# jmduarte/gnn-fpga

Hardware: AMD Instinct MI355X
Metric: edges/sec (EdgeNet+NodeNet fwd) on 100k-edge TrackML graphs; % HBM roofline (higher is better)
Workload: dtype f32; 1 GPU; c3 synthetic TrackML ACTS graphs: 256 graphs/launch/GPU x (10k hits, 100k segments), F=3, D=8, 3 MP iterations + final edge pass, index form resident in HBM; graphs_per_gpu=256, hits_per_graph=10000, segments_per_graph=100000

## Files before the change

gnn-fpga_amd/csrc/sell_pipeline.hip:

```cpp
#include "common.h"

#include <cstdlib>
#include <type_traits>
#include <utility>

namespace {
using namespace gnn;

constexpr int SLICE = 16;
constexpr int DESC = 8;

template <int F, int D>
struct TL {
    static constexpr int d4 = D / 4, C = F + D;
    static constexpr int a4(int x) { return (x + 3) & ~3; }
    static constexpr int o_w2 = 0;
    static constexpr int o_in = a4(o_w2 + d4);
    static constexpr int in_sz = d4 + F * d4;
    static constexpr int o_4 = a4(o_in + in_sz);
    static constexpr int w4_sz = d4 + D * d4;
    static constexpr int o_m = a4(o_4 + w4_sz);
    static constexpr int m_sz = d4 + C * d4;
    static constexpr int m_st = a4(m_sz);
    static constexpr int o_b2 = o_m + 5 * m_st;
// ... 40 lines not shown
            const int k = (t - d4) / d4, i = (t - d4) % d4;
            v = p.W4[(q * d4 + i) * D + k];
        }
    } else if (pos >= L::o_m && pos < L::o_b2 && (pos - L::o_m) % L::m_st < L::m_sz) {
        const int t = pos - L::o_m, m = t / L::m_st, u = t % L::m_st;
        if (u < d4) {
            const int r = q * d4 + u;
            v = (m == 0) ? kTwoLog2e * p.b1[r] : (m == 4) ? p.b3[r] : 0.0f;
        } else {
            const int k = (u - d4) / d4, r = q * d4 + (u - d4) % d4;
            switch (m) {
            case 0: v = kTwoLog2e * p.W1[r * 2 * C + k]; break;
            case 1: v = p.W3[r * 3 * C + k]; break;
            case 2: v = kTwoLog2e * p.W1[r * 2 * C + C + k]; break;
            case 3: v = p.W3[r * 3 * C + C + k]; break;
            default: v = p.W3[r * 3 * C + 2 * C + k]; break;
            }
        }
    } else if (pos == L::o_b2) {
        float sw = p.b2[0];
        for (int k = 0; k < D; ++k) sw += p.W2[k];
        v = -kLog2e * sw;
    }
    return v;
}

template <int F, int D, bool XP>
__device__ __forceinline__ void write_null_rows(const gnn_params_t &p, float *PRa, float *PRb,
                                                float *QSa, float *QSb, float *U, float *Pc,
                                                float *Qc, int64_t n_hits)
{
    constexpr int d4 = D / 4;
    for (int t = threadIdx.x; t < 2 * D; t += 256) {
        const int q = t / (2 * d4), w = t % (2 * d4);
        float pv = (w < d4) ? kTwoLog2e * p.b1[q * d4 + w] : 0.0f;
        if (XP && w < d4) pv = __builtin_amdgcn_exp2f(pv);
        const float qv = (XP && w < d4) ? 1.0f : 0.0f;
        PRa[n_hits * 2 * D + t] = pv;
        PRb[n_hits * 2 * D + t] = pv;
        QSa[n_hits * 2 * D + t] = qv;
        QSb[n_hits * 2 * D + t] = qv;
    }
    for (int t = threadIdx.x; t < D; t += 256) {
        U[n_hits * D + t] = 0.0f;
        const float pb = kTwoLog2e * p.b1[t];
        Pc[n_hits * D + t] = XP ? __builtin_amdgcn_exp2f(pb) : pb;
        Qc[n_hits * D + t] = XP ? 1.0f : 0.0f;
    }
}

template <int F, int D, bool XP>
__global__ __launch_bounds__(256) void k_pack(gnn_params_t p, float *__restrict__ table,
                                              float *PRa, float *PRb, float *QSa, float *QSb,
                                              float *U, float *Pc, float *Qc, int64_t n_hits)
{
    using L = TL<F, D>;
    for (int idx = blockIdx.x * 256 + threadIdx.x; idx < L::total; idx += gridDim.x * 256)
        table[idx] = table_entry<F, D>(p, idx);
    if (blockIdx.x == 0) write_null_rows<F, D, XP>(p, PRa, PRb, QSa, QSb, U, Pc, Qc, n_hits);
}

template <int CTRL>
__device__ __forceinline__ float dpp(float v)
{
    return __builtin_bit_cast(
        float, __builtin_amdgcn_mov_dpp(__builtin_bit_cast(int, v), CTRL, 0xF, 0xF, true));
}

__device__ __forceinline__ float quad_sum(float v)
{
    v += dpp<0xB1>(v);
    v += dpp<0x4E>(v);
    return v;
}

template <int N>
__device__ __forceinline__ void quad_allgather(const float (&loc)[N], float *out)
{
#pragma unroll
    for (int i = 0; i < N; ++i) {
        out[0 * N + i] = dpp<0x00>(loc[i]);
        out[1 * N + i] = dpp<0x55>(loc[i]);
        out[2 * N + i] = dpp<0xAA>(loc[i]);
        out[3 * N + i] = dpp<0xFF>(loc[i]);
    }
}

template <int N>
__device__ __forceinline__ void load_vec(const float *__restrict__ src, float *dst)
{
    if constexpr (N == 1) {
        dst[0] = src[0];
    } else if constexpr (N == 2) {
        const float2 v = *reinterpret_cast<const float2 *>(src);
        dst[0] = v.x; dst[1] = v.y;
    } else {
        static_assert(N % 4 == 0, "vector length");
#pragma unroll
        for (int i = 0; i < N / 4; ++i) {
            const float4 v = reinterpret_cast<const float4 *>(src)[i];
            dst[4 * i] = v.x; dst[4 * i + 1] = v.y; dst[4 * i + 2] = v.z; dst[4 * i + 3] = v.w;
        }
    }
}

typedef float f2_t __attribute__((ext_vector_type(2)));
typedef float f3_t __attribute__((ext_vector_type(3)));
typedef float f4_t __attribute__((ext_vector_type(4)));

template <int N>
__device__ __forceinline__ void store_vec(float *__restrict__ dst, const float *src)
{
    if constexpr (N == 1) {
        dst[0] = src[0];
    } else if constexpr (N == 2) {
        *reinterpret_cast<float2 *>(dst) = make_float2(src[0], src[1]);
    } else {
        static_assert(N % 4 == 0, "vector length");
#pragma unroll
        for (int i = 0; i < N / 4; ++i)
            reinterpret_cast<float4 *>(dst)[i] =
                make_float4(src[4 * i], src[4 * i + 1], src[4 * i + 2], src[4 * i + 3]);
    }
}

template <int NT>
__device__ __forceinline__ void stage4(const float *__restrict__ g, float *lds, int n4)
{
    const float4 *__restrict__ g4 = reinterpret_cast<const float4 *>(g);
    float4 *l4 = reinterpret_cast<float4 *>(lds);
    int i = threadIdx.x;
    for (; i + 7 * NT < n4; i += 8 * NT) {
        float4 v[8];
#pragma unroll
        for (int j = 0; j < 8; ++j) v[j] = g4[i + j * NT];
#pragma unroll
        for (int j = 0; j < 8; ++j) l4[i + j * NT] = v[j];
    }
    for (; i < n4; i += NT) l4[i] = g4[i];
}

template <int F, int D>
struct Cfg {
    static constexpr int NT = (D <= 16) ? 1024 : 256;
    static constexpr int lds_bytes = 160 * 1024;
    static constexpr int table_bytes = TL<F, D>::total * 4;
    static constexpr bool wide16 = (D == 16 && F <= 4);
    static constexpr int it_rec = (D <= 16 && !wide16) ? (lds_bytes - table_bytes - 2048) / (8 * D) : 0;
    static constexpr int ed_rec = (D <= 16) ? (lds_bytes - 2048) / (4 * D) : 0;
    static constexpr int tile_hits = (D <= 16 && !wide16) ? 1280 : 256;
    static constexpr int chunk_segments = 16384;
    static constexpr bool pipelined = (D <= 8 && F <= 3) || (D == 4);
    static constexpr bool iter2 = (D <= 8);
    static constexpr bool pack_first = (TL<F, D>::total > 4096);
    static constexpr bool fuse_first = iter2 && F <= 3 && !(F == 2 && D == 8);
};

template <int D4, int KD, int KF, bool PK = true>
__device__ __forceinline__ void role_gemv(const float *w, const float *hn, const float *x,
                                          float *out)
{
    constexpr int NW = D4 + (KD + KF) * D4;
    constexpr int CH = 8;
#ifndef GNN_NO_GEMV_PK
    if constexpr (PK && D4 >= 8 && D4 % 4 == 0) {
        const f4_t *wv = reinterpret_cast<const f4_t *>(__builtin_assume_aligned(w, 16));
        asm volatile("" ::: "memory");
        f2_t o2[D4 / 2];
#pragma unroll
        for (int v = 0; v < D4 / 4; ++v) {
            const f4_t t = wv[v];
            o2[2 * v] = f2_t{t.x, t.y};
            o2[2 * v + 1] = f2_t{t.z, t.w};
        }
        f4_t cur[D4 / 4], nxt[D4 / 4];
#pragma unroll
        for (int v = 0; v < D4 / 4; ++v) cur[v] = wv[D4 / 4 + v];
#pragma unroll
        for (int k = 0; k < KD + KF; ++k) {
            if (k + 1 < KD + KF)
#pragma unroll
                for (int v = 0; v < D4 / 4; ++v) nxt[v] = wv[(D4 + (k + 1) * D4) / 4 + v];
            const float in = k < KD ? hn[k < KD ? k : 0] : x[k >= KD ? k - KD : 0];
            const f2_t in2 = {in, in};
#pragma unroll
            for (int v = 0; v < D4 / 4; ++v) {
                o2[2 * v] = f2_t{cur[v].x, cur[v].y} * in2 + o2[2 * v];
                o2[2 * v + 1] = f2_t{cur[v].z, cur[v].w} * in2 + o2[2 * v + 1];
            }
#pragma unroll
            for (int v = 0; v < D4 / 4; ++v) cur[v] = nxt[v];
        }
#pragma unroll
        for (int i = 0; i < D4 / 2; ++i) {
            out[2 * i] = o2[i].x;
            out[2 * i + 1] = o2[i].y;
        }
        return;
    }
#endif
    const float4 *w4 = reinterpret_cast<const float4 *>(__builtin_assume_aligned(w, 16));
#pragma unroll
    for (int c0 = 0; c0 < NW; c0 += CH) {
        constexpr int dummy = 0; (void)dummy;
        float wr[CH];
#pragma unroll
        for (int v = 0; v < CH / 4; ++v) {
            if (c0 + 4 * v < NW) {
                const float4 t = w4[c0 / 4 + v];
                wr[4 * v] = t.x; wr[4 * v + 1] = t.y; wr[4 * v + 2] = t.z; wr[4 * v + 3] = t.w;
            }
        }
#pragma unroll
        for (int j = 0; j < CH; ++j) {
            const int g = c0 + j;
            if (g < NW) {
                if (g < D4) {
                    out[g] = wr[j];
                } else {
                    const int k = (g - D4) / D4, i = (g - D4) % D4;
                    out[i] = fmaf(wr[j], k < KD ? hn[k < KD ? k : 0] : x[k >= KD ? k - KD : 0], out[i]);
                }
            }
        }
    }
}

template <int KD, int KF>
__device__ __forceinline__ void role_gemv_burst(const float *w, const float *hn, const float *x,
                                                float *out)
{
    constexpr int NW = 2 + (KD + KF) * 2, NV = (NW + 3) / 4;
    const f4_t *wv = reinterpret_cast<const f4_t *>(__builtin_assume_aligned(w, 16));
    f4_t t[NV];
#pragma unroll
    for (int v = 0; v < NV; ++v) t[v] = wv[v];
    f2_t acc = {t[0].x, t[0].y};
#pragma unroll
    for (int j = 1; j < NW / 2; ++j) {
        const int k = j - 1;
        const float in = k < KD ? hn[k < KD ? k : 0] : x[k >= KD ? k - KD : 0];
        const f2_t wk = (j & 1) ? f2_t{t[j / 2].z, t[j / 2].w} : f2_t{t[j / 2].x, t[j / 2].y};
        acc = wk * f2_t{in, in} + acc;
    }
    out[0] = acc.x;
    out[1] = acc.y;
}

template <int F, int D, bool LAST, bool XP>
struct Records {
    static constexpr int d4 = D / 4;
    float pr[LAST ? d4 : 2 * d4], qs[LAST ? d4 : 2 * d4], u[d4];

    __device__ __forceinline__ void compute(const float *wl, const float *hn, const float *x)
    {
        using L = TL<F, D>;
        if constexpr (LAST) {
            role_gemv<d4, D, F>(wl + L::o_m + 0 * L::m_st, hn, x, pr);
            role_gemv<d4, D, F>(wl + L::o_m + 2 * L::m_st, hn, x, qs);
        } else {
            role_gemv<d4, D, F>(wl + L::o_m + 0 * L::m_st, hn, x, pr);
            role_gemv<d4, D, F>(wl + L::o_m + 1 * L::m_st, hn, x, pr + d4);
            role_gemv<d4, D, F>(wl + L::o_m + 2 * L::m_st, hn, x, qs);
            role_gemv<d4, D, F>(wl + L::o_m + 3 * L::m_st, hn, x, qs + d4);
            role_gemv<d4, D, F>(wl + L::o_m + 4 * L::m_st, hn, x, u);
        }
        if constexpr (XP) {
#pragma unroll
            for (int i = 0; i < d4; ++i) {
                pr[i] = __builtin_amdgcn_exp2f(pr[i]);
                qs[i] = __builtin_amdgcn_exp2f(qs[i]);
            }
        }
    }
    __device__ __forceinline__ void store(int64_t n, int q, float *__restrict__ PRn,
                                          float *__restrict__ QSn, float *__restrict__ U,
                                          float *__restrict__ Pc, float *__restrict__ Qc) const
    {
        if constexpr (LAST) {
            store_vec<d4>(Pc + n * D + q * d4, pr);
            store_vec<d4>(Qc + n * D + q * d4, qs);
        } else {
            store_vec<2 * d4>(PRn + n * 2 * D + q * 2 * d4, pr);
            store_vec<2 * d4>(QSn + n * 2 * D + q * 2 * d4, qs);
            store_vec<d4>(U + n * D + q * d4, u);
        }
    }
};

template <int F, int D, bool LAST, bool XP, bool PK = true>
__device__ __forceinline__ void emit_to(const float *wl, const float *hn, const float *x,
                                        float *__restrict__ pr_dst, float *__restrict__ qs_dst,
                                        float *__restrict__ u_dst)
{
    using L = TL<F, D>;
    constexpr int d4 = D / 4;
    {
        float pr[LAST ? d4 : 2 * d4];
        role_gemv<d4, D, F, PK>(wl + L::o_m + 0 * L::m_st, hn, x, pr);
        if constexpr (XP)
#pragma unroll
            for (int i = 0; i < d4; ++i) pr[i] = __builtin_amdgcn_exp2f(pr[i]);
        if constexpr (!LAST) role_gemv<d4, D, F, PK>(wl + L::o_m + 1 * L::m_st, hn, x, pr + d4);
        store_vec<LAST ? d4 : 2 * d4>(pr_dst, pr);
    }
    {
// ... 694 lines not shown
}
template <int J>
__device__ __forceinline__ float quad_bcast_f(float v)
{
    return dpp<J * 0x55>(v);
}

constexpr int MAXC = 6;

template <int D>
struct Recs {
    float r[4][2 * (D / 4)];
    __device__ __forceinline__ void read(int cur, const float *REC, int q)
    {
        constexpr int d4 = D / 4;
        const int nb[4] = {quad_bcast_i<0>(cur), quad_bcast_i<1>(cur), quad_bcast_i<2>(cur),
                           quad_bcast_i<3>(cur)};
#ifdef GNN_ABLATE_LDS
#pragma unroll
        for (int j = 0; j < 4; ++j)
#pragma unroll
            for (int i = 0; i < 2 * d4; ++i) r[j][i] = __int_as_float(nb[j] + i);
        (void)REC;
#else
#pragma unroll
        for (int j = 0; j < 4; ++j) load_vec<2 * d4>(REC + (int64_t)nb[j] * 2 * D + q * 2 * d4, r[j]);
#endif
    }
};

__device__ __forceinline__ float bf_lo(unsigned w) { return __uint_as_float(w << 16); }
__device__ __forceinline__ float bf_hi(unsigned w) { return __uint_as_float(w & 0xFFFF0000u); }

template <int D4, bool XP, bool ES = false>
__device__ __forceinline__ void score4(const float (*rec)[2 * D4], const float *own,
                                       const float *w2, float b2, int q, float *acc, float *eo = nullptr,
                                       bool ok = false)
{
    float part[4];
#ifndef GNN_NO_PK
    constexpr bool use_pk = (D4 == 2), use_pk_wide = (D4 >= 8 && D4 % 2 == 0);
#else
    constexpr bool use_pk = false, use_pk_wide = false;
#endif
    if constexpr (use_pk) {
        const f2_t o2 = {own[0], own[1]}, one2 = {1.0f, 1.0f};
        float r[4][2];
#pragma unroll
        for (int j = 0; j < 4; ++j) {
            const f2_t pj = {rec[j][0], rec[j][1]};
            f2_t a;
            if constexpr (XP) {
                a = pj * o2 + one2;
            } else {
                const f2_t z = pj + o2;
                const f2_t ex = {__builtin_amdgcn_exp2f(z.x), __builtin_amdgcn_exp2f(z.y)};
                a = ex + one2;
            }
            r[j][0] = __builtin_amdgcn_rcpf(a.x);
            r[j][1] = __builtin_amdgcn_rcpf(a.y);
        }
        const f2_t wa = {w2[0], w2[0]}, wb = {w2[1], w2[1]};
        const f2_t p01 = wa * f2_t{r[0][0], r[1][0]} + wb * f2_t{r[0][1], r[1][1]};
        const f2_t p23 = wa * f2_t{r[2][0], r[3][0]} + wb * f2_t{r[2][1], r[3][1]};
        part[0] = p01.x; part[1] = p01.y; part[2] = p23.x; part[3] = p23.y;
    } else if constexpr (use_pk_wide) {
        const f2_t one2 = {1.0f, 1.0f};
#pragma unroll
        for (int j = 0; j < 4; ++j) {
            f2_t pj = {0.0f, 0.0f};
#pragma unroll
            for (int i = 0; i < D4; i += 2) {
                const f2_t rj = {rec[j][i], rec[j][i + 1]}, o2 = {own[i], own[i + 1]};
                f2_t a;
                if constexpr (XP) {
                    a = rj * o2 + one2;
                } else {
                    const f2_t z = rj + o2;
                    const f2_t ex = {__builtin_amdgcn_exp2f(z.x), __builtin_amdgcn_exp2f(z.y)};
                    a = ex + one2;
                }
                const f2_t r = {__builtin_amdgcn_rcpf(a.x), __builtin_amdgcn_rcpf(a.y)};
                pj = f2_t{w2[i], w2[i + 1]} * r + pj;
            }
            part[j] = pj.x + pj.y;
        }
    } else {
#pragma unroll
        for (int j = 0; j < 4; ++j) {
            part[j] = 0.0f;
#pragma unroll
            for (int i = 0; i < D4; ++i) {
                const float r = XP ? __builtin_amdgcn_rcpf(fmaf(rec[j][i], own[i], 1.0f))
                                   : r_f(rec[j][i] + own[i]);
                part[j] = fmaf(w2[i], r, part[j]);
            }
        }
    }
    const bool odd = q & 1, hi = q & 2;
    const float s0 = odd ? part[0] : part[1], s1 = odd ? part[2] : part[3];
    const float k0 = odd ? part[1] : part[0], k1 = odd ? part[3] : part[2];
    const float t0 = k0 + dpp<0xB1>(s0), t1 = k1 + dpp<0xB1>(s1);
    const float give = hi ? t0 : t1, keep = hi ? t1 : t0;
    const float mine = keep + dpp<0x4E>(give);
    const float e = r_f(mine + b2);
    if constexpr (ES)
        if (ok) *eo = e;
    const float e4[4] = {quad_bcast_f<0>(e), quad_bcast_f<1>(e), quad_bcast_f<2>(e),
                         quad_bcast_f<3>(e)};
    if constexpr (use_pk_wide) {
#pragma unroll
        for (int j = 0; j < 4; ++j) {
            const f2_t e2 = {e4[j], e4[j]};
#pragma unroll
            for (int i = 0; i < D4; i += 2) {
                const f2_t a2 = f2_t{rec[j][D4 + i], rec[j][D4 + i + 1]} * e2 + f2_t{acc[i], acc[i + 1]};
                acc[i] = a2.x;
                acc[i + 1] = a2.y;
            }
        }
    } else {
#pragma unroll
        for (int j = 0; j < 4; ++j)
#pragma unroll
            for (int i = 0; i < D4; ++i) acc[i] = fmaf(e4[j], rec[j][D4 + i], acc[i]);
    }
}

template <int D, bool XP, bool ES = false>
__device__ __forceinline__ void sweep(const int *pre, const int32_t *__restrict__ lst, int len,
                                      int null_idx, const float *REC, int q, const float *own,
                                      const float *w2, float b2, float *acc, float *ebase = nullptr, int elen = 0)
{
    constexpr int d4 = D / 4;
    if (len <= 0) return;
    auto fix = [&](int cur, int rem) {
        const int lim = rem < 4 ? rem : 4;
        return (q < lim) ? cur : null_idx;
    };
    Recs<D> a;
#pragma unroll
    for (int c = 0; c < MAXC; ++c) {
        if (4 * c < len) {
            a.read(fix(pre[c], len - 4 * c), REC, q);
            score4<d4, XP, ES>(a.r, own, w2, b2, q, acc, ebase + 4 * c + q, 4 * c + q < elen);
        }
    }
    for (int k = 4 * MAXC; k < len; k += 4) {
        a.read(fix(lst[k * SLICE], len - k), REC, q);
        score4<d4, XP, ES>(a.r, own, w2, b2, q, acc, ebase + k + q, k + q < elen);
    }
}

template <int D, int NC, bool XP, bool PIPE>
__device__ __forceinline__ void sweep16(int (&c)[NC], const int32_t *__restrict__ nbr16,
                                        const int32_t *__restrict__ off16, int slice, int i16,
                                        int len, const float *REC, int q, const float *own,
                                        const float *w2, float b2, float *acc)
{
    constexpr int d4 = D / 4;
    if (len <= 0) return;
    int taken = 0;
    auto take_word = [&]() {
        int w = c[0];
        if (taken >= NC) {
            a_load_i32_s<0>(w, nbr16 + __builtin_amdgcn_readfirstlane(off16[slice]) + taken * 4 * SLICE,
                            (unsigned)(q * SLICE + i16) * 4u);
            a_wait_all();
            asm volatile("" : "+v"(w));
        }
#pragma unroll
        for (int i = 0; i + 1 < NC; ++i) c[i] = c[i + 1];
        ++taken;
        return w;
    };
    typedef __attribute__((address_space(3))) const float lds_cf;
    const unsigned rec0 = (unsigned)(uintptr_t)(lds_cf *)(REC + q * 2 * d4);
    auto issue = [&](float (*r)[2 * d4], int w, bool hi) {
        const int wa = hi ? quad_bcast_i<2>(w) : quad_bcast_i<0>(w);
        const int wb = hi ? quad_bcast_i<3>(w) : quad_bcast_i<1>(w);
        unsigned ad[4];
        static_assert(8 * D <= 64, "record size must be an inline constant");
        asm("v_mad_u32_u16 %0, %1, %2, %3" : "=v"(ad[0]) : "v"(wa), "n"(8 * D), "v"(rec0));
        asm("v_mad_u32_u16 %0, %1, %2, %3 op_sel:[1,0,0,0]" : "=v"(ad[1]) : "v"(wa), "n"(8 * D), "v"(rec0));
        asm("v_mad_u32_u16 %0, %1, %2, %3" : "=v"(ad[2]) : "v"(wb), "n"(8 * D), "v"(rec0));
        asm("v_mad_u32_u16 %0, %1, %2, %3 op_sel:[1,0,0,0]" : "=v"(ad[3]) : "v"(wb), "n"(8 * D), "v"(rec0));
#pragma unroll
        for (int j = 0; j < 4; ++j) {
            if constexpr (d4 == 2) {
                const f4_t v = *(const __attribute__((address_space(3))) f4_t *)(uintptr_t)ad[j];
                r[j][0] = v.x; r[j][1] = v.y; r[j][2] = v.z; r[j][3] = v.w;
            } else {
                const f2_t v = *(const __attribute__((address_space(3))) f2_t *)(uintptr_t)ad[j];
                r[j][0] = v.x; r[j][1] = v.y;
            }
        }
    };
    static_assert(d4 == 1 || d4 == 2, "record piece is 8 or 16 bytes");
    if constexpr (!PIPE) {
        for (int k = 0; k < len; k += 8) {
            const int w = take_word();
            float r[4][2 * d4];
            issue(r, w, false);
            score4<d4, XP>(r, own, w2, b2, q, acc);
            if (k + 4 < len) {
                issue(r, w, true);
                score4<d4, XP>(r, own, w2, b2, q, acc);
            }
        }
        return;
    }
    float ra[4][2 * d4], rb[4][2 * d4];
    int w = take_word();
    issue(ra, w, false);
    for (int k = 0; k < len; k += 8) {
        const bool has_hi = k + 4 < len;
        if (has_hi) issue(rb, w, true);
        score4<d4, XP>(ra, own, w2, b2, q, acc);
        if (has_hi) {
            if (k + 8 < len) {
                w = take_word();
                issue(ra, w, false);
            }
            score4<d4, XP>(rb, own, w2, b2, q, acc);
        }
    }
}

struct TrainOut {
    const int32_t *seg_ptr;
    float *e_t, *Q_t, *H_next;
    int ldh;
};

template <int F, int D, bool LAST, bool XP, bool TR = false>
__global__ __launch_bounds__((Cfg<F, D>::NT)) void k_iter(
    const float *__restrict__ X, const float *__restrict__ table,
    const int32_t *__restrict__ tiles, const int32_t *__restrict__ in_off,
    const int32_t *__restrict__ in_nbr, const int32_t *__restrict__ out_off,
    const int32_t *__restrict__ out_nbr, const float *__restrict__ PR,
    const float *__restrict__ QS, float *__restrict__ U, float *__restrict__ PRn,
    float *__restrict__ QSn, float *__restrict__ Pc, float *__restrict__ Qc, int64_t n_pad,
    int tiles_per_xcd, int n_tiles, int ablate, TrainOut tro = TrainOut{})
{
    using L = TL<F, D>;
    using G = Cfg<F, D>;
    constexpr int d4 = L::d4, NT = G::NT;
    (void)tro;
    extern __shared__ __attribute__((aligned(16))) float smem[];
    float *lds = smem, *win = smem + L::total;
    stage4<NT>(table, lds, L::total / 4);

    const int tile = (blockIdx.x & 7) * tiles_per_xcd + (blockIdx.x >> 3);
    if (tile >= n_tiles) return;
    const int32_t *td = tiles + (int64_t)tile * DESC;
    const int s_begin = td[0], s_end = td[1], in_lo = td[2], in_cnt = td[3], out_lo = td[4],
              out_cnt = td[5], mode = td[6];
    const int lane = threadIdx.x & 63;
    const int q = lane & 3, i16 = lane >> 2;

    struct Pre {
        int il, ol, ib, ob;
        int cin[MAXC], cout[MAXC];
        AVec<d4> Pn, Qn;
        AVec<d4> acc;
        AVec<F> x;
    };
    auto prefetch = [&](Pre &p, int slice) {
        if (ablate & 8) { p.il = 12; p.ol = 12; p.ib = 0; p.ob = 0;
#pragma unroll
            for (int c = 0; c < MAXC; ++c) { p.cin[c] = 0; p.cout[c] = 0; }
            return; }
        p.ib = __builtin_amdgcn_readfirstlane(in_off[slice]);
        p.il = (__builtin_amdgcn_readfirstlane(in_off[slice + 1]) - p.ib) >> 4;
        p.ob = __builtin_amdgcn_readfirstlane(out_off[slice]);
        p.ol = (__builtin_amdgcn_readfirstlane(out_off[slice + 1]) - p.ob) >> 4;
        const int32_t *li = in_nbr + p.ib + q * SLICE + i16;
        const int32_t *lo = out_nbr + p.ob + q * SLICE + i16;
#define GNN_PF(C_)                                                              \
        if (4 * C_ < p.il) a_load_i32<C_ * 4 * SLICE * 4>(p.cin[C_], li);           \
        if (4 * C_ < p.ol) a_load_i32<C_ * 4 * SLICE * 4>(p.cout[C_], lo);
        GNN_PF(0) GNN_PF(1) GNN_PF(2) GNN_PF(3) GNN_PF(4) GNN_PF(5)
#undef GNN_PF
        static_assert(MAXC == 6, "prefetch is written out for 6 chunks");
        const int64_t n = (int64_t)slice * SLICE + i16;
        p.Pn.load(PR + n * 2 * D + q * 2 * d4);
        p.Qn.load(QS + n * 2 * D + q * 2 * d4);
        p.acc.load(U + n * D + q * d4);
        p.x.load(X + n * F);
    };
    auto arrive = [&](Pre &p) {
        a_wait_all();
        a_fence(p.cin); a_fence(p.cout);
        p.Pn.fence(); p.Qn.fence(); p.acc.fence(); p.x.fence();
    };
    constexpr int NWV = NT / 64;
    const int wv = threadIdx.x >> 6;
    const int rounds = (s_end - s_begin + NWV - 1) / NWV;
    auto slice_of = [&](int r) {
        const int sl = s_begin + r * NWV + ((r & 1) ? NWV - 1 - wv : wv);
        return (r < rounds && sl < s_end) ? sl : -1;
    };
    Pre cur, nxt;
    int slice = slice_of(0);
    if (slice >= 0) prefetch(cur, slice);
    float *winA = win, *winB = win + (in_cnt + 1) * 2 * D;
    if (G::it_rec > 0 && mode && !(ablate & 1)) {
        stage4<NT>(PR + (int64_t)in_lo * 2 * D, winA, in_cnt * 2 * D / 4);
        stage4<NT>(PR + n_pad * 2 * D, winA + in_cnt * 2 * D, 2 * D / 4);
        stage4<NT>(QS + (int64_t)out_lo * 2 * D, winB, out_cnt * 2 * D / 4);
        stage4<NT>(QS + n_pad * 2 * D, winB + out_cnt * 2 * D, 2 * D / 4);
    }
    __syncthreads();
    if (slice >= 0) arrive(cur);
    float w2[d4];
#pragma unroll
    for (int i = 0; i < d4; ++i) w2[i] = lds[q * L::stride + L::o_w2 + i];
    const float b2 = lds[L::o_b2];

    for (int r = 0; r < rounds; ++r) {
        const int next = slice_of(r + 1);
        if (next >= 0) {
            prefetch(nxt, next);
            if constexpr (!G::pipelined || TR) arrive(nxt);
        }
        Records<F, D, LAST, XP> rec;
        const int64_t n = (int64_t)slice * SLICE + i16;
        if (slice >= 0) {
            int woff = q * L::stride;
            asm volatile("" : "+v"(woff));
            const float *wl = lds + woff;
            float acc[d4], Pn[d4], Qn[d4], xv[F];
            cur.acc.get(acc); cur.x.get(xv);
            cur.Pn.get(Pn); cur.Qn.get(Qn);
            float *eb = nullptr;
            int en = 0;
            if constexpr (TR) {
                const int s0 = tro.seg_ptr[n];
                en = tro.seg_ptr[n + 1] - s0;
                eb = tro.e_t + s0;
            }
            if (ablate & 2) {
            } else if (G::it_rec > 0 && mode) {
                sweep<D, XP, TR>(cur.cin, in_nbr + cur.ib + q * SLICE + i16, cur.il, in_cnt, winA, q, Qn, w2, b2, acc, eb, en);
                sweep<D, XP>(cur.cout, out_nbr + cur.ob + q * SLICE + i16, cur.ol, out_cnt, winB, q, Pn, w2, b2, acc);
            } else {
                sweep<D, XP, TR>(cur.cin, in_nbr + cur.ib + q * SLICE + i16, cur.il, (int)n_pad, PR, q, Qn, w2, b2, acc, eb, en);
                sweep<D, XP>(cur.cout, out_nbr + cur.ob + q * SLICE + i16, cur.ol, (int)n_pad, QS, q, Pn, w2, b2, acc);
            }
            float ql[d4], qa[D];
#pragma unroll
            for (int i = 0; i < d4; ++i) ql[i] = tanh_f(acc[i]);
            if constexpr (TR) store_vec<d4>(tro.Q_t + n * D + q * d4, ql);
            quad_allgather<d4>(ql, qa);
            float hl[d4];
            role_gemv<d4, D, 0>(wl + L::o_4, qa, qa, hl);
#pragma unroll
            for (int i = 0; i < d4; ++i) hl[i] = tanh_f(hl[i]);
            if constexpr (TR) {
                float *hr = tro.H_next + n * tro.ldh;
                store_vec<d4>(hr + q * d4, hl);
                if (q == 0) {
#pragma unroll
                    for (int k = 0; k < F; ++k) hr[D + k] = xv[k];
                    for (int k = D + F; k < tro.ldh; ++k) hr[k] = 0.0f;
                }
            }
            float hn[D];
            quad_allgather<d4>(hl, hn);
            if (!(ablate & 4)) rec.compute(wl, hn, xv);
        }
        if constexpr (G::pipelined)
            if (next >= 0) arrive(nxt);
        cur = nxt;
        if (slice >= 0 && !(ablate & 16)) rec.store(n, q, PRn, QSn, U, Pc, Qc);
        slice = next;
    }
}

// ... 767 lines not shown
#pragma unroll
            for (int k = 0; k < F; ++k) x[k] = live ? xb[h * F + k] : 0.0f;
            round_fence(r);
            if (!live) continue;
            h0_of(wl, x, hn);
            if constexpr (d4 == 2) {
                role_gemv_burst<D, F>(wl + L::o_m + (2 * M) * L::m_st, hn, x, rec);
                role_gemv_burst<D, F>(wl + L::o_m + (2 * M + 1) * L::m_st, hn, x, rec + d4);
            } else {
                role_gemv<d4, D, F>(wl + L::o_m + (2 * M) * L::m_st, hn, x, rec);
                role_gemv<d4, D, F>(wl + L::o_m + (2 * M + 1) * L::m_st, hn, x, rec + d4);
            }
            if constexpr (XP)
#pragma unroll
                for (int i = 0; i < d4; ++i) rec[i] = __builtin_amdgcn_exp2f(rec[i]);
            store_vec<2 * d4>(buf + h * 2 * D + q * 2 * d4, rec);
        }
        null_fence();
        put_null(buf, cnt, which);
    };

    struct PreA0 { int len; int c[NC]; AVec<d4> Q, U; };
    constexpr bool XPRE = F <= 4;
    struct PreB0 { int len; int c[NC]; AVec<d4> P; AVec<XPRE ? F : 0> x; };
    struct PreX { int len; int c[NC]; AVec<F> x; };
    using PreA = std::conditional_t<FIRST, PreX, PreA0>;
    using PreB = std::conditional_t<FIRST, PreX, PreB0>;
    const unsigned lo_list = (unsigned)(q * SLICE + i16) * 4u;
    const unsigned lo_rec = (unsigned)(i16 * 2 * D + q * 2 * d4) * 4u;
    const unsigned lo_vec = (unsigned)(i16 * D + q * d4) * 4u;
    const unsigned lo_x = (unsigned)(i16 * F) * 4u;
    auto prefetchA = [&](PreA &p, int slice_) {
        const int slice = __builtin_amdgcn_readfirstlane(slice_);
        p.len = (__builtin_amdgcn_readfirstlane(in_off[slice + 1]) -
                 __builtin_amdgcn_readfirstlane(in_off[slice])) >> 4;
        const int32_t *li = in_nbr16 + __builtin_amdgcn_readfirstlane(in_off16[slice]);
#define GNN_PF(C_) if (8 * C_ < p.len) a_load_i32_s<C_ * 4 * SLICE * 4>(p.c[C_], li, lo_list);
        GNN_PF(0) GNN_PF(1) GNN_PF(2)
#undef GNN_PF
        const int64_t n0 = (int64_t)slice * SLICE;
        if constexpr (FIRST) {
            p.x.load_s(X + n0 * F, lo_x);
        } else {
            p.Q.load_s(QS + n0 * 2 * D, lo_rec);
            p.U.load_s(U + n0 * D, lo_vec);
        }
    };
    auto prefetchB = [&](PreB &p, int slice_) {
        const int slice = __builtin_amdgcn_readfirstlane(slice_);
        p.len = (__builtin_amdgcn_readfirstlane(out_off[slice + 1]) -
                 __builtin_amdgcn_readfirstlane(out_off[slice])) >> 4;
        const int32_t *lo = out_nbr16 + __builtin_amdgcn_readfirstlane(out_off16[slice]);
#define GNN_PF(C_) if (8 * C_ < p.len) a_load_i32_s<C_ * 4 * SLICE * 4>(p.c[C_], lo, lo_list);
        GNN_PF(0) GNN_PF(1) GNN_PF(2)
#undef GNN_PF
        static_assert(NC == 3, "prefetch is written out for 3 words (24 steps)");
        const int64_t n0 = (int64_t)slice * SLICE;
        if constexpr (!FIRST) p.P.load_s(PR + n0 * 2 * D, lo_rec);
        if constexpr (XPRE || FIRST) p.x.load_s(X + n0 * F, lo_x);
    };
    auto arriveA = [&](PreA &p) {
        a_wait_all();
        a_fence(p.c);
        if constexpr (FIRST) {
            p.x.fence();
        } else {
            p.Q.fence();
            p.U.fence();
        }
    };
    auto arriveB = [&](PreB &p) {
        a_wait_all();
        a_fence(p.c);
        if constexpr (!FIRST) p.P.fence();
        if constexpr (XPRE || FIRST) p.x.fence();
    };

    constexpr int MAXR = 5;
    float ac0[d4], ac1[d4], ac2[d4], ac3[d4], ac4[d4];
    auto acc_put = [&](int r, const float *a) {
#pragma unroll
        for (int i = 0; i < d4; ++i) {
            ac0[i] = (r == 0) ? a[i] : ac0[i];
            ac1[i] = (r == 1) ? a[i] : ac1[i];
            ac2[i] = (r == 2) ? a[i] : ac2[i];
            ac3[i] = (r == 3) ? a[i] : ac3[i];
            ac4[i] = (r >= 4) ? a[i] : ac4[i];
        }
    };
    auto acc_get = [&](int r, float *a) {
#pragma unroll
        for (int i = 0; i < d4; ++i)
            a[i] = (r == 0) ? ac0[i] : (r == 1) ? ac1[i] : (r == 2) ? ac2[i] : (r == 3) ? ac3[i] : ac4[i];
    };
    static_assert(MAXR == 5, "accumulator slots are written out for 5 rounds");
#pragma unroll
    for (int i = 0; i < d4; ++i) ac0[i] = ac1[i] = ac2[i] = ac3[i] = ac4[i] = 0.0f;

    Desc d = load_desc(tile);
    PreA a_cur, a_nxt;
    PreB b_cur, b_nxt;
    if constexpr (FIRST) {
        xstage_issue(d.in_lo, d.in_cnt, bufA, capA);
        if (slice_a(d, 0) >= 0) prefetchA(a_cur, slice_a(d, 0));
        compute_window(bufA, d.in_cnt, capA, WinA{});
    } else {
        stage_issue(PR + (int64_t)d.in_lo * 2 * D, bufA, d.in_cnt);
        if (slice_a(d, 0) >= 0) prefetchA(a_cur, slice_a(d, 0));
        __syncthreads();
        stage_commit(bufA, d.in_cnt, WinA{});
    }
    if (slice_a(d, 0) >= 0) arriveA(a_cur);

    float w2[d4];
    for (;;) {
        __syncthreads();
#pragma unroll
        for (int i = 0; i < d4; ++i) w2[i] = lds[q * L::stride + L::o_w2 + i];
        const float b2 = lds[L::o_b2];
        const int rounds = (d.s_end - d.s_begin + NWV - 1) / NWV;
        if constexpr (FIRST)
            xstage_issue(d.out_lo, d.out_cnt, bufB, capB);
        else
            stage_issue(QS + (int64_t)d.out_lo * 2 * D, bufB, d.out_cnt);
        auto roundA = [&](int r, auto lr) {
            constexpr bool LR = decltype(lr)::value;
            const int slice = slice_a(d, r);
            const int next = LR ? -1 : slice_a(d, r + 1);
            if constexpr (LR) {
                if (slice_a(d, 0) >= 0) prefetchB(b_cur, slice_a(d, 0));
            } else {
                if (next >= 0) prefetchA(a_nxt, next);
            }
            float acc[d4];
            if (slice >= 0) {
                float Qn[d4];
                if constexpr (FIRST) {
                    int woff = q * L::stride;
                    asm volatile("" : "+v"(woff));
                    const float *wl = lds + woff;
                    float xo[F], h0[D];
                    a_cur.x.get(xo);
                    h0_of(wl, xo, h0);
                    role_gemv<d4, D, F>(wl + L::o_m + 2 * L::m_st, h0, xo, Qn);
                    if constexpr (XP)
#pragma unroll
                        for (int i = 0; i < d4; ++i) Qn[i] = __builtin_amdgcn_exp2f(Qn[i]);
                    role_gemv<d4, D, F>(wl + L::o_m + 4 * L::m_st, h0, xo, acc);
                } else {
                    a_cur.U.get(acc);
                    a_cur.Q.get(Qn);
                }
                const int len = __builtin_amdgcn_readfirstlane(a_cur.len);
                sweep16<D, NC, XP, !FIRST>(a_cur.c, in_nbr16, in_off16, slice, i16, len, bufA, q, Qn, w2, b2, acc);
            }
            if constexpr (!LR) {
                if (next >= 0) {
                    arriveA(a_nxt);
                    a_cur = a_nxt;
                }
            }
            if (slice >= 0) acc_put(r, acc);
        };
        for (int r = 0; r + 1 < rounds; ++r) roundA(r, std::false_type{});
        roundA(rounds - 1, std::true_type{});
        if constexpr (FIRST)
            compute_window(bufB, d.out_cnt, capB, WinB{});
        else
            stage_commit(bufB, d.out_cnt, WinB{});
        if (slice_a(d, 0) >= 0) arriveB(b_cur);
        __syncthreads();
        const int tnext = tile + gridDim.x;
        Desc dn = d;
        if (tnext < n_tiles) {
            dn = load_desc(tnext);
            if constexpr (FIRST)
                xstage_issue(dn.in_lo, dn.in_cnt, bufA, capA);
            else
                stage_issue(PR + (int64_t)dn.in_lo * 2 * D, bufA, dn.in_cnt);
        }
        auto roundB = [&](int r, auto lr) {
            constexpr bool LR = decltype(lr)::value;
            const int slice = slice_a(d, r);
            const int next = LR ? -1 : slice_a(d, r + 1);
            if constexpr (LR) {
                if (tnext < n_tiles && slice_a(dn, 0) >= 0) prefetchA(a_cur, slice_a(dn, 0));
            } else {
                if (next >= 0) prefetchB(b_nxt, next);
            }
            float xv[F], acc[d4];
            if (slice >= 0) {
                float Pn[d4];
                acc_get(r, acc);
                if constexpr (XPRE || FIRST) {
                    b_cur.x.get(xv);
                } else {
                    const float *xr = X + ((int64_t)__builtin_amdgcn_readfirstlane(slice) * SLICE + i16) * F;
#pragma unroll
                    for (int k = 0; k < F; ++k) xv[k] = xr[k];
                }
                if constexpr (FIRST) {
                    int woff = q * L::stride;
                    asm volatile("" : "+v"(woff));
                    const float *wl = lds + woff;
                    float h0[D];
                    h0_of(wl, xv, h0);
                    role_gemv<d4, D, F>(wl + L::o_m + 0 * L::m_st, h0, xv, Pn);
                    if constexpr (XP)
#pragma unroll
                        for (int i = 0; i < d4; ++i) Pn[i] = __builtin_amdgcn_exp2f(Pn[i]);
                } else {
                    b_cur.P.get(Pn);
                }
                const int len = __builtin_amdgcn_readfirstlane(b_cur.len);
                sweep16<D, NC, XP, false>(b_cur.c, out_nbr16, out_off16, slice, i16, len, bufB, q, Pn, w2, b2, acc);
            }
            if constexpr (!LR) {
                if (next >= 0) {
                    arriveB(b_nxt);
                    b_cur = b_nxt;
                }
            }
            if constexpr (D == 8) {
                if (slice >= 0) {
                    using MTL = MT<F, D>;
                    typedef float f4v __attribute__((ext_vector_type(4)));
                    const float *mb = mt + MTL::o_b;
                    const int hit = lane & 15, g = lane >> 4;
                    const int from = ((hit << 2) | g) << 2;
                    const float q0 = __int_as_float(__builtin_amdgcn_ds_bpermute(from, __float_as_int(tanh_f(acc[0]))));
                    const float q1 = __int_as_float(__builtin_amdgcn_ds_bpermute(from, __float_as_int(tanh_f(acc[1]))));
                    float xm[F];
#pragma unroll
                    for (int k = 0; k < F; ++k)
                        xm[k] = __int_as_float(__builtin_amdgcn_ds_bpermute(hit << 4, __float_as_int(xv[k])));
                    f4v h = *reinterpret_cast<const f4v *>(mb + 64 + 4 * g);
                    h = __builtin_amdgcn_mfma_f32_16x16x4f32(mt[MTL::o_w4 + lane], q0, h, 0, 0, 0);
                    h = __builtin_amdgcn_mfma_f32_16x16x4f32(mt[MTL::o_w4 + 64 + lane], q1, h, 0, 0, 0);
                    const float hh[4] = {tanh_f(h.x), tanh_f(h.y), tanh_f(h.z), tanh_f(h.w)};
                    float h3a = 0.0f, h3b = 0.0f;
                    if constexpr (MTL::PACK) {
                        h3a = __int_as_float(__builtin_amdgcn_ds_bpermute(hit << 2, __float_as_int(hh[3])));
                        h3b = __int_as_float(__builtin_amdgcn_ds_bpermute((16 + hit) << 2, __float_as_int(hh[3])));
                    }
                    auto slot_in = [&](int st) {
                        if constexpr (MTL::PACK) {
                            if (g < 2) return hh[st];
                            if (g == 2) return st == 0 ? h3a : st == 1 ? h3b : (0 < F ? xm[0] : 0.0f);
                            float v = 0.0f;
#pragma unroll
                            for (int k = 1; k < F; ++k) v = (k == 1 + st) ? xm[k] : v;
                            return v;
                        }
                        if (st < 4) {
                            if (g < 2) return hh[st];
                            float v = 0.0f;
#pragma unroll
                            for (int k = 0; k < F; ++k)
                                if (k == st || k == 4 + st) v = (g == (k < 4 ? 2 : 3) && (k & 3) == st) ? xm[k] : v;
                            return v;
                        }
                        float v = 0.0f;
#pragma unroll
                        for (int k = 8; k < F; ++k) v = (g == k - 8) ? xm[k] : v;
                        return v;
                    };
                    float bin_[MTL::NS];
#pragma unroll
                    for (int st = 0; st < MTL::NS; ++st) bin_[st] = slot_in(st);
                    const int64_t n = (int64_t)__builtin_amdgcn_readfirstlane(slice) * SLICE + hit;
                    constexpr int NP = LAST ? 1 : 3;
#pragma unroll
                    for (int T = 0; T < NP; ++T) {
                        f4v c = *reinterpret_cast<const f4v *>(mb + 16 * (1 + T) + 4 * g);
#pragma unroll
                        for (int st = 0; st < MTL::NS; ++st)
                            c = __builtin_amdgcn_mfma_f32_16x16x4f32(mt[MTL::o_t + MTL::t_sz * T + 64 * st + lane],
                                                                     bin_[st], c, 0, 0, 0);
                        if constexpr (LAST) {
                            if constexpr (XP) {
                                c.x = __builtin_amdgcn_exp2f(c.x); c.y = __builtin_amdgcn_exp2f(c.y);
                                c.z = __builtin_amdgcn_exp2f(c.z); c.w = __builtin_amdgcn_exp2f(c.w);
                            }
                            *reinterpret_cast<f4v *>((g < 2 ? Pc : Qc) + n * D + 4 * (g & 1)) = c;
                        } else if (T < 2) {
                            if constexpr (XP) {
                                c.x = __builtin_amdgcn_exp2f(c.x);
                                c.y = __builtin_amdgcn_exp2f(c.y);
                            }
                            *reinterpret_cast<f4v *>((T == 0 ? PRn : QSn) + n * 2 * D + 4 * g) = c;
                        } else if (g < 2) {
                            *reinterpret_cast<f4v *>(U + n * D + 4 * g) = c;
                        }
                    }
                }
            } else if (slice >= 0) {
                int woff = q * L::stride;
                asm volatile("" : "+v"(woff));
                const float *wl = lds + woff;
                float ql[d4], qa[D], hl[d4], hn[D];
#pragma unroll
                for (int i = 0; i < d4; ++i) ql[i] = tanh_f(acc[i]);
                quad_allgather<d4>(ql, qa);
                role_gemv<d4, D, 0>(wl + L::o_4, qa, qa, hl);
#pragma unroll
                for (int i = 0; i < d4; ++i) hl[i] = tanh_f(hl[i]);
                quad_allgather<d4>(hl, hn);
                const int64_t n0 = (int64_t)__builtin_amdgcn_readfirstlane(slice) * SLICE;
                auto at = [](float *base, unsigned off) {
                    return reinterpret_cast<float *>(reinterpret_cast<char *>(base) + off);
                };
                if constexpr (LAST)
                    emit_to<F, D, LAST, XP>(wl, hn, xv, at(Pc + n0 * D, lo_vec), at(Qc + n0 * D, lo_vec), nullptr);
                else
                    emit_to<F, D, LAST, XP>(wl, hn, xv, at(PRn + n0 * 2 * D, lo_rec), at(QSn + n0 * 2 * D, lo_rec),
                                            at(U + n0 * D, lo_vec));
            }
        };
        for (int r = 0; r + 1 < rounds; ++r) roundB(r, std::false_type{});
        roundB(rounds - 1, std::true_type{});
        if (tnext >= n_tiles) break;
        if constexpr (FIRST)
            compute_window(bufA, dn.in_cnt, capA, WinA{});
        else
            stage_commit(bufA, dn.in_cnt, WinA{});
        if (slice_a(dn, 0) >= 0) arriveA(a_cur);
        tile = tnext;
        d = dn;
    }
}

template <int F, int D, bool XP>
__global__ __launch_bounds__((Cfg<F, D>::NT)) void k_edge(
    const int32_t *__restrict__ chunks, const int32_t *__restrict__ src,
    const int32_t *__restrict__ dst, const int32_t *__restrict__ sd16,
    const float *__restrict__ Pc, const float *__restrict__ Qc,
    const float *__restrict__ table, float *__restrict__ e, int64_t n_pad, int chunks_per_xcd,
    int n_chunks, int backward)
{
    using G = Cfg<F, D>;
    const float *__restrict__ W2 = table + TL<F, D>::o_flat;
    constexpr int NT = G::NT;
    extern __shared__ __attribute__((aligned(16))) float win[];
    const int pos = (blockIdx.x & 7) * chunks_per_xcd + (blockIdx.x >> 3);
    if (pos >= n_chunks) return;
    const int chunk = backward ? n_chunks - 1 - pos : pos;
    const int32_t *cd = chunks + (int64_t)chunk * DESC;
    const int e0 = cd[0], e1 = cd[1], s_lo = cd[2], s_cnt = cd[3], d_lo = cd[4], d_cnt = cd[5],
              mode = cd[6];
    float *winA = win, *winB = win + (s_cnt + 1) * D;
    if (G::ed_rec > 0 && mode) {
        stage4<NT>(Pc + (int64_t)s_lo * D, winA, s_cnt * D / 4);
        stage4<NT>(Pc + n_pad * D, winA + s_cnt * D, D / 4);
        stage4<NT>(Qc + (int64_t)d_lo * D, winB, d_cnt * D / 4);
        stage4<NT>(Qc + n_pad * D, winB + d_cnt * D, D / 4);
        __syncthreads();
    }
    const float b2 = W2[D];
    auto score = [&](const float *p, const float *qq) {
        float acc = b2;
#pragma unroll
        for (int k = 0; k < D; ++k)
            acc = fmaf(W2[k], XP ? __builtin_amdgcn_rcpf(fmaf(p[k], qq[k], 1.0f)) : r_f(p[k] + qq[k]), acc);
        return r_f(acc);
    };
    if (G::ed_rec > 0 && mode) {
        constexpr int B8 = 8;
        for (int j0 = e0 + (int)threadIdx.x; j0 < e1; j0 += B8 * NT) {
// ... 548 lines not shown
```

Baseline: 31.10 billion edges/s.

## Add lane-rotated neighbor sweep for D=8 non-first message-passing iterations

Adds sweep16_lane, an alternative inner sweep for D=8 that gives each lane of a quad a rotated 4-float chunk of the neighbor record. Each lane does one 16-byte LDS load per chunk instead of four broadcast loads of full records. The edge score is reduced across chunks in registers, and the per-chunk sums are combined at the end with DPP rotations. This is meant to cut redundant LDS traffic and address math in the hot sweep. In exchange it adds cross-lane shuffles and a less pipelined loop that no longer double-buffers the record loads.

```diff
diff --git a/gnn-fpga_amd/csrc/sell_pipeline.hip b/gnn-fpga_amd/csrc/sell_pipeline.hip
--- a/gnn-fpga_amd/csrc/sell_pipeline.hip
+++ b/gnn-fpga_amd/csrc/sell_pipeline.hip
@@ -216,6 +216,11 @@
     static constexpr int chunk_segments = 16384;
     static constexpr bool pipelined = (D <= 8 && F <= 3) || (D == 4);
     static constexpr bool iter2 = (D <= 8);
+#ifdef GNN_QUAD_SWEEP
+    template <bool FIRST, bool PHASE_B> static constexpr bool lane_sweep = false;
+#else
+    template <bool FIRST, bool PHASE_B> static constexpr bool lane_sweep = iter2 && D == 8 && !FIRST;
+#endif
     static constexpr bool pack_first = (TL<F, D>::total > 4096);
     static constexpr bool fuse_first = iter2 && F <= 3 && !(F == 2 && D == 8);
 };
@@ -1216,6 +1221,23 @@
     }
 }
 
+template <int NC>
+__device__ __forceinline__ int take_word16(int (&c)[NC], int &taken, const int32_t *__restrict__ nbr16,
+                                           const int32_t *__restrict__ off16, int slice, int i16, int q)
+{
+    int w = c[0];
+    if (taken >= NC) {
+        a_load_i32_s<0>(w, nbr16 + __builtin_amdgcn_readfirstlane(off16[slice]) + taken * 4 * SLICE,
+                        (unsigned)(q * SLICE + i16) * 4u);
+        a_wait_all();
+        asm volatile("" : "+v"(w));
+    }
+#pragma unroll
+    for (int i = 0; i + 1 < NC; ++i) c[i] = c[i + 1];
+    ++taken;
+    return w;
+}
+
 template <int D, int NC, bool XP, bool PIPE>
 __device__ __forceinline__ void sweep16(int (&c)[NC], const int32_t *__restrict__ nbr16,
                                         const int32_t *__restrict__ off16, int slice, int i16,
@@ -1225,19 +1247,7 @@
     constexpr int d4 = D / 4;
     if (len <= 0) return;
     int taken = 0;
-    auto take_word = [&]() {
-        int w = c[0];
-        if (taken >= NC) {
-            a_load_i32_s<0>(w, nbr16 + __builtin_amdgcn_readfirstlane(off16[slice]) + taken * 4 * SLICE,
-                            (unsigned)(q * SLICE + i16) * 4u);
-            a_wait_all();
-            asm volatile("" : "+v"(w));
-        }
-#pragma unroll
-        for (int i = 0; i + 1 < NC; ++i) c[i] = c[i + 1];
-        ++taken;
-        return w;
-    };
+    auto take_word = [&]() { return take_word16<NC>(c, taken, nbr16, off16, slice, i16, q); };
     typedef __attribute__((address_space(3))) const float lds_cf;
     const unsigned rec0 = (unsigned)(uintptr_t)(lds_cf *)(REC + q * 2 * d4);
     auto issue = [&](float (*r)[2 * d4], int w, bool hi) {
@@ -1289,6 +1299,78 @@
             score4<d4, XP>(rb, own, w2, b2, q, acc);
         }
     }
+}
+
+template <int NC, bool XP>
+__device__ __forceinline__ void sweep16_lane(int (&c)[NC], const int32_t *__restrict__ nbr16,
+                                             const int32_t *__restrict__ off16, int slice, int i16,
+                                             int len, const float *REC, int q, const float *own,
+                                             const float *wtab, int wst, float b2, float *acc)
+{
+    constexpr int D = 8, CH = 4;
+    if (len <= 0) return;
+    int taken = 0;
+    auto take_word = [&]() { return take_word16<NC>(c, taken, nbr16, off16, slice, i16, q); };
+    typedef __attribute__((address_space(3))) const float lds_cf;
+    f2_t ownr[4], w2r[4], sum[4];
+    unsigned base[4];
+    ownr[0] = f2_t{own[0], own[1]};
+    ownr[1] = f2_t{dpp<0x39>(own[0]), dpp<0x39>(own[1])};
+    ownr[2] = f2_t{dpp<0x4E>(own[0]), dpp<0x4E>(own[1])};
+    ownr[3] = f2_t{dpp<0x93>(own[0]), dpp<0x93>(own[1])};
+#pragma unroll
+    for (int s = 0; s < 4; ++s) {
+        const int ch = (s + q) & 3;
+        base[s] = (unsigned)(uintptr_t)(lds_cf *)(REC + ch * CH);
+        w2r[s] = f2_t{wtab[ch * wst], wtab[ch * wst + 1]};
+        sum[s] = f2_t{0.0f, 0.0f};
+    }
+    const unsigned sh = (q & 1) << 4;
+    auto issue = [&](f4_t *r, int w, bool hi) {
+        const int wq = hi ? __builtin_amdgcn_mov_dpp(w, 0xFA, 0xF, 0xF, true)
+                          : __builtin_amdgcn_mov_dpp(w, 0x50, 0xF, 0xF, true);
+        const unsigned idx = (unsigned)wq >> sh;
+#pragma unroll
+        for (int s = 0; s < 4; ++s) {
+            unsigned ad;
+            asm("v_mad_u32_u16 %0, %1, %2, %3" : "=v"(ad) : "v"(idx), "n"(8 * D), "v"(base[s]));
+            r[s] = *(const __attribute__((address_space(3))) f4_t *)(uintptr_t)ad;
+        }
+    };
+    auto score = [&](const f4_t *r) {
+        const f2_t one2 = {1.0f, 1.0f};
+        f2_t z2 = {b2, 0.0f};
+#pragma unroll
+        for (int s = 0; s < 4; ++s) {
+            const f2_t ps = {r[s].x, r[s].y};
+            f2_t a;
+            if constexpr (XP) {
+                a = ps * ownr[s] + one2;
+            } else {
+                const f2_t z = ps + ownr[s];
+                const f2_t ex = {__builtin_amdgcn_exp2f(z.x), __builtin_amdgcn_exp2f(z.y)};
+                a = ex + one2;
+            }
+            const f2_t rr = {__builtin_amdgcn_rcpf(a.x), __builtin_amdgcn_rcpf(a.y)};
+            z2 = w2r[s] * rr + z2;
+        }
+        const float e = r_f(z2.x + z2.y);
+        const f2_t e2 = {e, e};
+#pragma unroll
+        for (int s = 0; s < 4; ++s) sum[s] = f2_t{r[s].z, r[s].w} * e2 + sum[s];
+    };
+    for (int k = 0; k < len; k += 8) {
+        const int w = take_word();
+        f4_t r[4];
+        issue(r, w, false);
+        score(r);
+        if (k + 4 < len) {
+            issue(r, w, true);
+            score(r);
+        }
+    }
+    acc[0] += (sum[0].x + dpp<0x93>(sum[1].x)) + (dpp<0x4E>(sum[2].x) + dpp<0x39>(sum[3].x));
+    acc[1] += (sum[0].y + dpp<0x93>(sum[1].y)) + (dpp<0x4E>(sum[2].y) + dpp<0x39>(sum[3].y));
 }
 
 struct TrainOut {
@@ -2362,7 +2444,11 @@
                     a_cur.Q.get(Qn);
                 }
                 const int len = __builtin_amdgcn_readfirstlane(a_cur.len);
-                sweep16<D, NC, XP, !FIRST>(a_cur.c, in_nbr16, in_off16, slice, i16, len, bufA, q, Qn, w2, b2, acc);
+                if constexpr (Cfg<F, D>::template lane_sweep<FIRST, false>)
+                    sweep16_lane<NC, XP>(a_cur.c, in_nbr16, in_off16, slice, i16, len, bufA, q, Qn,
+                                                    lds + L::o_w2, L::stride, b2, acc);
+                else
+                    sweep16<D, NC, XP, !FIRST>(a_cur.c, in_nbr16, in_off16, slice, i16, len, bufA, q, Qn, w2, b2, acc);
             }
             if constexpr (!LR) {
                 if (next >= 0) {
@@ -2423,7 +2509,11 @@
                     b_cur.P.get(Pn);
                 }
                 const int len = __builtin_amdgcn_readfirstlane(b_cur.len);
-                sweep16<D, NC, XP, false>(b_cur.c, out_nbr16, out_off16, slice, i16, len, bufB, q, Pn, w2, b2, acc);
+                if constexpr (Cfg<F, D>::template lane_sweep<FIRST, true>)
+                    sweep16_lane<NC, XP>(b_cur.c, out_nbr16, out_off16, slice, i16, len, bufB, q, Pn,
+                                                   lds + L::o_w2, L::stride, b2, acc);
+                else
+                    sweep16<D, NC, XP, false>(b_cur.c, out_nbr16, out_off16, slice, i16, len, bufB, q, Pn, w2, b2, acc);
             }
             if constexpr (!LR) {
                 if (next >= 0) {
```

Result: faster. 32.04 billion edges/s, median of 6 (+3.0%).
